# tudelft-iv/CCVPE

Measured on NVIDIA B200. Metric: VIGOR pairs/sec (CVM_VIGOR forward + pose decode, 320x640 panorama + 512x512 aerial), higher is better.
Workload: dtype bf16

## Files before the change

### ccvpe_b200/build.py

```python
from __future__ import annotations

import concurrent.futures
import os
import shutil
import subprocess
import sys

PKG_DIR = os.path.dirname(os.path.abspath(__file__))
CSRC = os.path.join(PKG_DIR, "csrc")
OBJ_DIR = os.path.join(PKG_DIR, "build")
INCLUDE = os.path.join(os.path.dirname(PKG_DIR), "include")
LIB_PATH = os.path.join(PKG_DIR, "libccvpe_b200.so")
SOURCES = ["runtime.cu", "descriptors.cu", "match.cu", "pointwise.cu", "igemm_simt.cu", "igemm_tcgen05.cu",
           "conv_ring_tcgen05.cu", "match_tcgen05.cu", "project_tcgen05.cu", "stem_tcgen05.cu", "encoder_ops.cu", "ingest.cu", "train_ops.cu", "wgrad_tcgen05.cu"]
NVCC_FLAGS = ["-gencode", "arch=compute_100a,code=sm_100a", "-lineinfo", "-O3", "-std=c++17", "-Xcompiler", "-fPIC"]


def _nvcc() -> str:
    for cand in (os.environ.get("NVCC"), shutil.which("nvcc"), "/usr/local/cuda/bin/nvcc"):
        if cand and os.path.exists(cand):
            return cand
    raise RuntimeError("nvcc not found; libccvpe_b200.so cannot be built")


def _headers():
    return [os.path.join(CSRC, f) for f in os.listdir(CSRC) if f.endswith((".cuh", ".h"))] + \
           [os.path.join(INCLUDE, "ccvpe_b200.h")]


def _sources():
    return [s for s in SOURCES if os.path.exists(os.path.join(CSRC, s))]


def stale() -> bool:
    if not os.path.exists(LIB_PATH):
        return True
    t = os.path.getmtime(LIB_PATH)
# ... 40 lines not shown
```

### ccvpe_b200/cabi.py

```python
from __future__ import annotations

import ctypes as C
import os
from typing import Optional, Sequence

import torch

from . import build as _build

F32, BF16 = 0, 1
ABI_VERSION = 3
SE_SUM_SCALE = 1048576.0
BACKEND_AUTO, BACKEND_SIMT, BACKEND_TCGEN05 = 0, 1, 2

EXPORTED_SYMBOLS = (
    "ccvpe_abi_version", "ccvpe_last_error", "ccvpe_launch_count", "ccvpe_reset_launch_count",
    "ccvpe_grd_descriptor", "ccvpe_grd_descriptors", "ccvpe_igemm", "ccvpe_igemm_plan", "ccvpe_match_scratch_elems", "ccvpe_match_plan", "ccvpe_match_level",
    "ccvpe_softmax_scratch_elems", "ccvpe_softmax_heatmap", "ccvpe_ori_normalize",
    "ccvpe_pose_scratch_bytes", "ccvpe_pose_decode", "ccvpe_bias_silu_nhwc", "ccvpe_dwconv_bias_silu_nhwc",
    "ccvpe_pointwise_silu_nhwc", "ccvpe_stem_conv_silu_nhwc", "ccvpe_se_gate_scale", "ccvpe_mbconv_project_nhwc",
    "ccvpe_wrap_columns_nhwc",
    "ccvpe_ingest_u8", "ccvpe_stem_conv_silu_u8_nhwc",
    "ccvpe_wgrad_workspace_elems", "ccvpe_wgrad", "ccvpe_wgrad_plan", "ccvpe_colsum_workspace_elems", "ccvpe_colsum",
    "ccvpe_relu_bwd", "ccvpe_scale_rows", "ccvpe_planar_to_cl", "ccvpe_cl_to_planar", "ccvpe_ori_normalize_bwd",
    "ccvpe_match_bwd_scratch_elems", "ccvpe_match_level_bwd", "ccvpe_loss_workspace_elems", "ccvpe_infonce_loss",
    "ccvpe_cross_entropy_loss", "ccvpe_orientation_loss", "ccvpe_grd_descriptors_bwd",
)


class CcvpeError(RuntimeError):
    pass


class IgemmDesc(C.Structure):
    _fields_ = [
        ("a0", C.c_void_p), ("a1", C.c_void_p),
        ("c0", C.c_int32), ("c1", C.c_int32), ("ld0", C.c_int32), ("ld1", C.c_int32),
        ("B", C.c_int32), ("Hin", C.c_int32), ("Win", C.c_int32), ("Hout", C.c_int32), ("Wout", C.c_int32),
        ("stride", C.c_int32), ("kh", C.c_int32), ("kw", C.c_int32), ("pad", C.c_int32),
        ("N", C.c_int32), ("dtype", C.c_int32),
        ("w_kn", C.c_void_p), ("w_nk", C.c_void_p),
        ("bias", C.c_void_p), ("row_scale", C.c_void_p), ("row_r1", C.c_void_p), ("r1_w", C.c_void_p),
        ("relu", C.c_int32), ("out_mode", C.c_int32), ("out_dtype", C.c_int32), ("ldo", C.c_int32),
        ("out", C.c_void_p),
# ... 75 lines not shown
    lib.ccvpe_bias_silu_nhwc.restype = C.c_int
    lib.ccvpe_bias_silu_nhwc.argtypes = [C.c_void_p, C.c_void_p, C.c_void_p, C.c_int64, C.c_int64, C.c_int64,
                                         C.c_int, C.c_int, C.c_int, C.c_int, C.c_void_p, C.c_void_p]
    lib.ccvpe_dwconv_bias_silu_nhwc.restype = C.c_int
    lib.ccvpe_dwconv_bias_silu_nhwc.argtypes = [C.c_void_p, C.c_int64, C.c_int64, C.c_int64, C.c_int, C.c_int,
                                                C.c_void_p, C.c_void_p, C.c_void_p, C.c_int, C.c_int, C.c_int, C.c_int,
                                                C.c_void_p, C.c_void_p]
    lib.ccvpe_pointwise_silu_nhwc.restype = C.c_int
    lib.ccvpe_pointwise_silu_nhwc.argtypes = [C.c_void_p, C.c_int, C.c_int, C.c_int, C.c_int, C.c_int, C.c_void_p,
                                              C.c_void_p, C.c_int, C.c_void_p, C.c_int, C.c_int, C.c_void_p]
    lib.ccvpe_stem_conv_silu_nhwc.restype = C.c_int
    lib.ccvpe_stem_conv_silu_nhwc.argtypes = [C.c_void_p, C.c_int, C.c_int, C.c_int, C.c_void_p, C.c_void_p, C.c_int,
                                              C.c_void_p, C.c_int, C.c_int, C.c_int, C.c_int, C.c_int, C.c_void_p]
    lib.ccvpe_stem_conv_silu_u8_nhwc.restype = C.c_int
    lib.ccvpe_stem_conv_silu_u8_nhwc.argtypes = [C.c_void_p, C.c_int, C.c_int, C.c_int, C.c_int, C.c_void_p,
                                                 C.POINTER(C.c_float), C.POINTER(C.c_float), C.c_void_p, C.c_void_p, C.c_int,
                                                 C.c_void_p, C.c_int, C.c_int, C.c_int, C.c_int, C.c_int, C.c_void_p]
    lib.ccvpe_se_gate_scale.restype = C.c_int
    lib.ccvpe_se_gate_scale.argtypes = [C.c_void_p, C.c_float] + [C.c_void_p] * 6 + [C.c_int] * 5 + [C.c_void_p] * 2
    lib.ccvpe_mbconv_project_nhwc.restype = C.c_int
    lib.ccvpe_mbconv_project_nhwc.argtypes = [C.c_void_p] * 6 + [C.c_int] * 4 + [C.c_void_p]
    lib.ccvpe_wrap_columns_nhwc.restype = C.c_int
    lib.ccvpe_wrap_columns_nhwc.argtypes = [C.c_void_p, C.c_int, C.c_int, C.c_int, C.c_int, C.c_int, C.c_int, C.c_void_p]
    lib.ccvpe_ingest_u8.restype = C.c_int
    lib.ccvpe_ingest_u8.argtypes = [C.c_void_p, C.c_int, C.c_int, C.c_int, C.c_int, C.c_int, C.c_void_p,
                                    C.POINTER(C.c_float), C.POINTER(C.c_float), C.c_void_p, C.c_void_p]
    lib.ccvpe_wgrad_workspace_elems.restype = C.c_int64
    lib.ccvpe_wgrad_workspace_elems.argtypes = [C.POINTER(WgradDesc)]
    lib.ccvpe_wgrad.restype = C.c_int
    lib.ccvpe_wgrad.argtypes = [C.POINTER(WgradDesc), C.c_void_p]
    lib.ccvpe_wgrad_plan.restype = C.c_int
    lib.ccvpe_wgrad_plan.argtypes = [C.POINTER(WgradDesc)]
    lib.ccvpe_colsum_workspace_elems.restype = C.c_int64
    lib.ccvpe_colsum_workspace_elems.argtypes = [C.c_int64, C.c_int, C.c_int]
    lib.ccvpe_colsum.restype = C.c_int
    lib.ccvpe_colsum.argtypes = [C.c_void_p, C.c_int, C.c_int, C.c_int, C.c_int, C.c_int, C.c_int, C.c_void_p, C.c_int,
                                 C.c_void_p, C.c_void_p, C.c_void_p]
    lib.ccvpe_relu_bwd.restype = C.c_int
    lib.ccvpe_relu_bwd.argtypes = [C.c_void_p, C.c_void_p, C.c_int, C.c_int64, C.c_void_p]
    lib.ccvpe_scale_rows.restype = C.c_int
    lib.ccvpe_scale_rows.argtypes = [C.c_void_p, C.c_int, C.c_void_p, C.c_void_p, C.c_int64, C.c_int, C.c_void_p]
    lib.ccvpe_planar_to_cl.restype = C.c_int
    lib.ccvpe_planar_to_cl.argtypes = [C.c_void_p, C.c_void_p, C.c_int, C.c_int, C.c_int, C.c_int64, C.c_int, C.c_void_p]
    lib.ccvpe_cl_to_planar.restype = C.c_int
    lib.ccvpe_cl_to_planar.argtypes = [C.c_void_p, C.c_int, C.c_void_p, C.c_int, C.c_int, C.c_int64, C.c_int, C.c_void_p]
    lib.ccvpe_ori_normalize_bwd.restype = C.c_int
# ... 202 lines not shown
                                       _ptr(chan_sum), _stream()), "ccvpe_bias_silu_nhwc")


def dwconv_bias_silu_nhwc(x_pad: torch.Tensor, w: torch.Tensor, bias: torch.Tensor, y: torch.Tensor, k: int, stride: int,
                          chan_sum: Optional[torch.Tensor] = None):
    _require_cuda(x_pad, w, bias, y, chan_sum)
    _check_se_sum(chan_sum)
    B, Hp, Wp, Cc = x_pad.shape
    if x_pad.stride(3) != 1 or not y.is_contiguous():
        raise CcvpeError("dwconv_bias_silu_nhwc: channels must be contiguous and y contiguous")
    _check(load().ccvpe_dwconv_bias_silu_nhwc(_ptr(x_pad), x_pad.stride(0), x_pad.stride(1), x_pad.stride(2), Hp, Wp,
                                              _ptr(w), _ptr(bias), _ptr(y), B, Cc, k, stride, _ptr(chan_sum), _stream()),
           "ccvpe_dwconv_bias_silu_nhwc")


def pad_k_blocks(w: torch.Tensor) -> torch.Tensor:
    N, K = w.shape
    kw = 16 if K <= 16 else (32 if K < 64 else 64)
    out = torch.zeros((N, -(-K // kw) * kw), dtype=torch.bfloat16, device=w.device)
    out[:, :K] = w
    return out.contiguous()


def pointwise_silu_nhwc(x: torch.Tensor, w_nk: torch.Tensor, bias: Optional[torch.Tensor], out: torch.Tensor,
                        pad_lo: int = 0, pad_hi: int = 0):
    _require_cuda(x, w_nk, bias, out)
    B, H, W, K = x.shape
    N = w_nk.shape[0]
    if not x.is_contiguous() or not out.is_contiguous() or x.dtype != torch.bfloat16 or out.dtype != torch.bfloat16:
        raise CcvpeError("pointwise_silu_nhwc: x and out must be contiguous bf16")
    if tuple(out.shape) != (B, H + pad_lo + pad_hi, W + pad_lo + pad_hi, N):
        raise CcvpeError(f"pointwise_silu_nhwc: out has shape {tuple(out.shape)}")
    if bias is not None and bias.dtype != torch.float32:
        raise CcvpeError("pointwise_silu_nhwc: bias must be fp32")
    _check(load().ccvpe_pointwise_silu_nhwc(_ptr(x), B, H, W, K, K, _ptr(w_nk), _ptr(bias), N, _ptr(out), pad_lo, pad_hi,
                                            _stream()), "ccvpe_pointwise_silu_nhwc")


def stem_conv_silu_nhwc(x: torch.Tensor, w: torch.Tensor, bias: torch.Tensor, out: torch.Tensor, in_pad_lo: int,
                        in_pad_hi: int, out_pad_lo: int, out_pad_hi: int, circular: bool):
    _require_cuda(x, w, bias, out)
    B, Cin, H, W = x.shape
    CO = w.shape[1]
    if Cin != 3 or x.dtype != torch.float32 or not x.is_contiguous() or w.dtype != torch.float32 or bias.dtype != torch.float32:
        raise CcvpeError("stem_conv_silu_nhwc: x must be contiguous fp32 [B,3,H,W], w / bias fp32")
    Ho, Wo = (H + in_pad_lo + in_pad_hi - 3) // 2 + 1, (W + in_pad_lo + in_pad_hi - 3) // 2 + 1
# ... 243 lines not shown
```

### ccvpe_b200/csrc/common.cuh

```cuda
#pragma once

#include <cuda_bf16.h>
#include <cuda_runtime.h>
#include <stdint.h>

#include <atomic>
#include <cstdarg>
#include <cstdio>

#include "../../include/ccvpe_b200.h"

namespace ccvpe {

char* last_error_buffer();
std::atomic<int64_t>& launch_counter();

inline int fail(int code, const char* fmt, ...) {
  va_list ap;
  va_start(ap, fmt);
  vsnprintf(last_error_buffer(), 512, fmt, ap);
  va_end(ap);
  return code;
}

// ... 67 lines not shown
  uint2 raw;
  raw.x = *reinterpret_cast<uint32_t*>(&lo);
  raw.y = *reinterpret_cast<uint32_t*>(&hi);
  *reinterpret_cast<uint2*>(p) = raw;
}

__device__ __forceinline__ uint64_t pack_f32x2(float lo, float hi) {
  uint64_t r;
  asm("mov.b64 %0, {%1, %2};" : "=l"(r) : "f"(lo), "f"(hi));
  return r;
}
__device__ __forceinline__ void unpack_f32x2(uint64_t v, float& lo, float& hi) {
  asm("mov.b64 {%0, %1}, %2;" : "=f"(lo), "=f"(hi) : "l"(v));
}
__device__ __forceinline__ uint64_t bf16x2_to_f32x2(uint32_t v) {
  return pack_f32x2(__uint_as_float(v << 16), __uint_as_float(v & 0xffff0000u));
}
__device__ __forceinline__ uint64_t ffma2(uint64_t a, uint64_t b, uint64_t c) {
  uint64_t d;
  asm("fma.rn.f32x2 %0, %1, %2, %3;" : "=l"(d) : "l"(a), "l"(b), "l"(c));
  return d;
}

__device__ __forceinline__ float warp_sum(float v) {
#pragma unroll
  for (int o = 16; o > 0; o >>= 1) v += __shfl_xor_sync(0xffffffffu, v, o);
  return v;
}
__device__ __forceinline__ float warp_max(float v) {
#pragma unroll
  for (int o = 16; o > 0; o >>= 1) v = fmaxf(v, __shfl_xor_sync(0xffffffffu, v, o));
  return v;
}

}
```

### ccvpe_b200/csrc/encoder_ops.cu

```cuda
#include <cstdlib>
#include <cstring>

#include "common.cuh"

namespace ccvpe {

constexpr float kSeFixedScale = 1048576.f;
__device__ __forceinline__ unsigned long long se_fixed(float v) {
  return (unsigned long long)__float2ll_rn(v * kSeFixedScale);
}

__global__ void __launch_bounds__(256)
bias_silu_nhwc_kernel(const __nv_bfloat16* __restrict__ x, const __nv_bfloat16* __restrict__ bias,
                      __nv_bfloat16* __restrict__ y, int64_t y_sb, int64_t y_sh, int64_t y_sw, int H, int W, int C,
                      int pix_per_block, long long* __restrict__ chan_sum) {
  extern __shared__ unsigned long long s_sum[];
  const int G = C >> 3;
  const int lanes = blockDim.x / G;
  const int cg = threadIdx.x % G, pl = threadIdx.x / G;
  const int b = blockIdx.y;
  const int HW = H * W;
  const int p_lo = blockIdx.x * pix_per_block;
  const int p_hi = min(HW, p_lo + pix_per_block);
  if (chan_sum) {
    for (int c = threadIdx.x; c < C; c += blockDim.x) s_sum[c] = 0ull;
    __syncthreads();
  }
  float bv[8] = {0.f, 0.f, 0.f, 0.f, 0.f, 0.f, 0.f, 0.f};
  if (bias && pl < lanes) {
    uint4 q = *reinterpret_cast<const uint4*>(bias + cg * 8);
    const __nv_bfloat162* h = reinterpret_cast<const __nv_bfloat162*>(&q);
#pragma unroll
    for (int j = 0; j < 4; ++j) {
// ... 804 lines not shown
```

### ccvpe_b200/fast_encoder.py

```python
from __future__ import annotations

from typing import Dict, List, Tuple

import torch
from torch.nn import functional as F

from . import cabi
from .efficientnet import EfficientNetB0, MBConv, SamePadConv2d


def _fold(conv: torch.nn.Conv2d, bn: torch.nn.BatchNorm2d) -> Tuple[torch.Tensor, torch.Tensor]:
    w = conv.weight.detach().float()
    scale = bn.weight.detach().float() / torch.sqrt(bn.running_var.detach().float() + bn.eps)
    bias = bn.bias.detach().float() - bn.running_mean.detach().float() * scale
    if conv.bias is not None:
        bias = bias + conv.bias.detach().float() * scale
    return w * scale.view(-1, 1, 1, 1), bias


class _Block:
    __slots__ = ("has_expand", "residual", "stride", "kernel", "pad_lo", "pad_hi", "w_exp", "b_exp", "w_exp_nk",
                 "b_exp_f32", "w_dw", "b_dw",
                 "w_red", "b_red", "w_se", "w_se_t", "b_se", "w_proj", "b_proj", "mid", "cout", "w_dw_taps")


class FastEncoder:
    def __init__(self, enc: EfficientNetB0, dtype: torch.dtype = torch.bfloat16):
        self.dtype = dtype
        self.circular = bool(enc._conv_stem._circular)
        dev = enc._conv_stem.weight.device
        cast = lambda t: t.to(device=dev, dtype=dtype).contiguous()
        w, b = _fold(enc._conv_stem, enc._bn0)
        self.stem_w = cast(w).contiguous(memory_format=torch.channels_last)
        self.stem_b = cast(b)
        self.stem_pad = (enc._conv_stem._pad_lo, enc._conv_stem._pad_hi)
        self.stem_w_taps = w.permute(1, 2, 3, 0).reshape(27, -1).to(device=dev, dtype=torch.float32).contiguous()
        self.stem_b_f32 = b.to(device=dev, dtype=torch.float32).contiguous()
        self.blocks: List[_Block] = []
        pending = None
        for blk in enc._blocks:
            assert isinstance(blk, MBConv)
            o = _Block()
            o.has_expand, o.residual = blk._has_expand, blk._residual
            dw: SamePadConv2d = blk._depthwise_conv
            o.stride, o.kernel = dw.stride[0], dw.kernel_size[0]
            o.pad_lo, o.pad_hi = dw._pad_lo, dw._pad_hi
            if o.has_expand:
                w, b = _fold(blk._expand_conv, blk._bn0)
                if pending is not None:
# ... 2 lines not shown
                o.w_exp_nk = cabi.pad_k_blocks(o.w_exp)
                o.b_exp_f32 = b.to(device=dev, dtype=torch.float32).contiguous()
            else:
                assert pending is None
                o.w_exp = o.b_exp = None
            w, b = _fold(dw, blk._bn1)
            o.w_dw, o.b_dw = cast(w).contiguous(memory_format=torch.channels_last), cast(b)
            o.mid = w.shape[0]
            o.w_dw_taps = cast(w.reshape(o.mid, -1).t())
            o.w_red, o.b_red = cast(blk._se_reduce.weight.detach().flatten(1)), cast(blk._se_reduce.bias.detach())
            o.w_se, o.b_se = cast(blk._se_expand.weight.detach().flatten(1)), cast(blk._se_expand.bias.detach())
            o.w_se_t = o.w_se.t().contiguous()
            w, b = _fold(blk._project_conv, blk._bn2)
            pending = b + (pending if (o.residual and pending is not None) else 0.0)
            o.w_proj, o.b_proj = cast(w.flatten(1)), cast(pending)
            o.cout = w.shape[0]
            self.blocks.append(o)
        w, b = _fold(enc._conv_head, enc._bn1)
        b = b + w.flatten(1) @ pending.to(w.device)
        self.head_w, self.head_b = cast(w.flatten(1)), cast(b)
        self.head_w_nk = cabi.pad_k_blocks(self.head_w)
        self.head_b_f32 = b.to(device=dev, dtype=torch.float32).contiguous()
        self._buffers: Dict[tuple, torch.Tensor] = {}
        self._mid_total = sum(o.mid for o in self.blocks)
        self.keep = set(range(len(self.blocks)))

    def _padded(self, B, C, H, W, lo, hi, tag) -> torch.Tensor:
        key = (tag, B, C, H, W, lo, hi)
        buf = self._buffers.get(key)
        if buf is None:
            buf = torch.zeros((B, H + lo + hi, W + lo + hi, C), dtype=self.dtype, device=self.stem_w.device)
            self._buffers[key] = buf
        return buf

    def _packed_bias(self, o, rep) -> torch.Tensor:
        key = ("bproj", id(o), rep)
        buf = self._buffers.get(key)
        if buf is None:
            buf = o.b_proj.repeat(rep).contiguous()
            self._buffers[key] = buf
        return buf

    def _wrap_columns(self, buf, H, W, lo, hi):
        if buf.is_cuda and buf.dtype == torch.bfloat16 and buf.is_contiguous():
            cabi.wrap_columns_nhwc(buf, H, W, lo, hi)
            return
        if lo:
            buf[:, lo:lo + H, :lo, :] = buf[:, lo:lo + H, W:W + lo, :]
        if hi:
            buf[:, lo:lo + H, lo + W:, :] = buf[:, lo:lo + H, lo:lo + hi, :]

    def _act(self, x_nhwc: torch.Tensor, bias, pad=None, want_sum: bool = False):
        B, H, W, C = x_nhwc.shape
        buf = None
        if pad is not None:
            lo, hi = pad
# ... 35 lines not shown
                cabi.stem_conv_silu_u8_nhwc(x.contiguous(), self.stem_w_taps, self.stem_b_f32, buf, lo, hi, o0.pad_lo,
                                            o0.pad_hi, self.circular)
            else:
                cabi.stem_conv_silu_nhwc(x.float().contiguous(), self.stem_w_taps, self.stem_b_f32, buf, lo, hi, o0.pad_lo,
                                         o0.pad_hi, self.circular)
            stem_padded = buf.permute(0, 3, 1, 2)
            pre = pre_bias = None
        else:
            if x.dtype == torch.uint8:
                raise cabi.CcvpeError("uint8 images are ingested by the CUDA bf16 encoder plan only (models.ingest otherwise)")
            x = x.to(dt).contiguous(memory_format=torch.channels_last)
            if self.circular:
                x = F.pad(F.pad(x, (lo, hi, 0, 0), mode="circular"), (0, 0, lo, hi))
            else:
                x = F.pad(x, (lo, hi, lo, hi))
            pre = F.conv2d(x, self.stem_w, None, stride=2).permute(0, 2, 3, 1)
            pre_bias = self.stem_b
        cur = None
        outs: List[torch.Tensor] = []
        sums_ws = torch.zeros(x.shape[0] * self._mid_total, dtype=torch.int64, device=x.device) if fused_dw else None
        sums_off = 0
        for o in self.blocks:
            dw_pad = (o.pad_lo, o.pad_hi) if (self.circular or o.stride == 2 or fused_dw) else None
            if stem_padded is not None:
                block_in = None
                mid_in_plain, mid_in_padded = None, stem_padded
                stem_padded = None
            elif pre is not None and not o.has_expand and not o.residual:
                plain, padded, _unused = self._act(pre, pre_bias, pad=dw_pad)
                block_in = None
                mid_in_plain, mid_in_padded = (plain if padded is None else None), padded
                pre = None
            else:
                if pre is not None:
                    cur = self._act(pre, pre_bias)[0]
                    pre = None
                block_in = cur
                B, H, W, Cin = cur.shape
                if o.has_expand and fused_dw:
                    buf = self._padded(B, o.mid, H, W, o.pad_lo, o.pad_hi, "dw")
                    cabi.pointwise_silu_nhwc(cur, o.w_exp_nk, o.b_exp_f32, buf, o.pad_lo, o.pad_hi)
                    if self.circular:
                        self._wrap_columns(buf, H, W, o.pad_lo, o.pad_hi)
                    mid_in_plain, mid_in_padded = None, buf.permute(0, 3, 1, 2)
                elif o.has_expand:
                    e = F.linear(cur.reshape(B * H * W, Cin), o.w_exp, o.b_exp).view(B, H, W, o.mid)
                    plain, padded, _unused = self._act(e, None, pad=dw_pad)
                    mid_in_plain, mid_in_padded = (plain if padded is None else None), padded
                else:
                    if dw_pad is not None:
                        buf = self._padded(B, o.mid, H, W, o.pad_lo, o.pad_hi, "dw")
                        buf[:, o.pad_lo:o.pad_lo + H, o.pad_lo:o.pad_lo + W, :] = cur
                        if self.circular:
                            self._wrap_columns(buf, H, W, o.pad_lo, o.pad_hi)
                        mid_in_plain, mid_in_padded = None, buf.permute(0, 3, 1, 2)
                    else:
                        mid_in_plain, mid_in_padded = cur, None
            if fused_dw:
                xp = mid_in_padded.permute(0, 2, 3, 1)
                Bp, Hp, Wp, _ = xp.shape
                Ho, Wo = (Hp - o.kernel) // o.stride + 1, (Wp - o.kernel) // o.stride + 1
                d = torch.empty((Bp, Ho, Wo, o.mid), dtype=dt, device=xp.device)
                sums = sums_ws[sums_off:sums_off + Bp * o.mid].view(Bp, o.mid)
                sums_off += Bp * o.mid
                cabi.dwconv_bias_silu_nhwc(xp, o.w_dw_taps, o.b_dw, d, o.kernel, o.stride, sums)
            else:
                if mid_in_padded is not None:
                    d = F.conv2d(mid_in_padded, o.w_dw, None, stride=o.stride, groups=o.mid)
                else:
                    d = F.conv2d(mid_in_plain.permute(0, 3, 1, 2), o.w_dw, None, stride=1, padding=o.pad_lo,
                                 groups=o.mid)
                d, _unused, sums = self._act(d.permute(0, 2, 3, 1), o.b_dw, want_sum=True)
            Bo, Ho, Wo, _ = d.shape
            if fused_dw:
                rep = 2 if (o.mid <= 32 and (Ho * Wo) % 2 == 0 and not o.residual) else 1
                wg = torch.empty((Bo, rep * o.cout, rep * o.mid), dtype=dt, device=d.device)
                gate_ws = torch.empty((Bo, o.mid), dtype=torch.float32, device=d.device)
                cabi.se_gate_scale(sums, 1.0 / float(Ho * Wo), o.w_red, o.b_red, o.w_se_t, o.b_se, o.w_proj, wg, gate_ws, rep)
            else:
                sq = (sums / float(Ho * Wo)).to(dt)
                g = torch.sigmoid(F.linear(F.silu(F.linear(sq, o.w_red, o.b_red)), o.w_se, o.b_se))
# ... 39 lines not shown
```

### include/ccvpe_b200.h

```cpp
#ifndef CCVPE_B200_H_
#define CCVPE_B200_H_

#include <stdint.h>

#ifdef __cplusplus
extern "C" {
#endif

#define CCVPE_ABI_VERSION 3

enum { CCVPE_F32 = 0, CCVPE_BF16 = 1 };

enum {
  CCVPE_OK = 0,
  CCVPE_ERR_BAD_ARGUMENT = -1,
  CCVPE_ERR_UNSUPPORTED = -2,
  CCVPE_ERR_CUDA = -3,
  CCVPE_ERR_NO_DEVICE = -4
};

enum {
  CCVPE_BACKEND_AUTO = 0,
  CCVPE_BACKEND_SIMT = 1,
  CCVPE_BACKEND_TCGEN05 = 2
// ... 61 lines not shown

int ccvpe_dwconv_bias_silu_nhwc(const void* x, int64_t x_sb, int64_t x_sh, int64_t x_sw, int Hp, int Wp,
                                const void* w, const void* bias, void* y, int B, int C, int K, int S,
                                int64_t* chan_sum, void* stream);

int ccvpe_stem_conv_silu_nhwc(const float* x, int B, int H, int W, const float* w, const float* bias, int CO,
                              void* out, int in_pad_lo, int in_pad_hi, int out_pad_lo, int out_pad_hi, int circular,
                              void* stream);

int ccvpe_stem_conv_silu_u8_nhwc(const uint8_t* x, int B, int H, int Wsrc, int crop_w, const int32_t* shift,
                                 const float* mean_host, const float* std_host, const float* w, const float* bias, int CO,
                                 void* out, int in_pad_lo, int in_pad_hi, int out_pad_lo, int out_pad_hi, int circular,
                                 void* stream);

int ccvpe_wrap_columns_nhwc(void* buf, int B, int H, int W, int C, int pad_lo, int pad_hi, void* stream);

int ccvpe_se_gate_scale(const int64_t* chan_sum, float inv_hw, const void* w_red, const void* b_red, const void* w_se,
                        const void* b_se, const void* w_proj, void* wg, int B, int mid, int R, int cout, int rep,
                        float* gate_ws, void* stream);

int ccvpe_pointwise_silu_nhwc(const void* x, int B, int H, int W, int K, int ldx, const void* w_nk, const float* bias,
                              int N, void* out, int pad_lo, int pad_hi, void* stream);

int ccvpe_mbconv_project_nhwc(const void* d, const void* wg, const void* residual, const void* bias, void* out,
                              void* out_biased, int B, int HW, int mid, int cout, void* stream);

int ccvpe_ingest_u8(const uint8_t* src, int nhwc, int B, int H, int W, int crop_w, const int32_t* shift,
                    const float* mean_host, const float* std_host, float* dst, void* stream);


typedef struct ccvpe_wgrad_desc {
  const void* a0; const void* a1;
  int32_t c0, c1, ld0, ld1;
  int32_t B, Hin, Win, Hout, Wout;
  int32_t stride, kh, kw, pad;
  const void* g; int32_t N, ldg;
  const float* g_row_scale;
  int32_t dtype;
  float* out;
  float* workspace; int64_t workspace_elems;
  int32_t backend;
} ccvpe_wgrad_desc;
int64_t ccvpe_wgrad_workspace_elems(const ccvpe_wgrad_desc* desc);
int ccvpe_wgrad(const ccvpe_wgrad_desc* desc, void* stream);
int ccvpe_wgrad_plan(const ccvpe_wgrad_desc* desc);

// ... 37 lines not shown
```

Baseline: 5958.

## Fuse MBConv expand 1x1 GEMM with depthwise conv in one tcgen05 kernel

Adds a persistent kernel that runs the 1x1 expansion GEMM on tcgen05 into TMEM, applies bias+SiLU, and writes rows into a shared-memory ring. Depthwise KxK conv, bias/SiLU and SE channel sums are then computed from that ring in the same kernel. This removes the round trip of the wide expanded activation through global memory and the separate launches for the early, narrow-input blocks. It costs heavy shared-memory use and redundant halo-row GEMM work between bands, and it applies only when Cin<=64 and mid is divisible by 48.

```diff
diff --git a/ccvpe_b200/build.py b/ccvpe_b200/build.py
--- a/ccvpe_b200/build.py
+++ b/ccvpe_b200/build.py
@@ -12,7 +12,7 @@
 INCLUDE = os.path.join(os.path.dirname(PKG_DIR), "include")
 LIB_PATH = os.path.join(PKG_DIR, "libccvpe_b200.so")
 SOURCES = ["runtime.cu", "descriptors.cu", "match.cu", "pointwise.cu", "igemm_simt.cu", "igemm_tcgen05.cu",
-           "conv_ring_tcgen05.cu", "match_tcgen05.cu", "project_tcgen05.cu", "stem_tcgen05.cu", "encoder_ops.cu", "ingest.cu", "train_ops.cu", "wgrad_tcgen05.cu"]
+           "conv_ring_tcgen05.cu", "match_tcgen05.cu", "project_tcgen05.cu", "stem_tcgen05.cu", "expand_dw_tcgen05.cu", "encoder_ops.cu", "ingest.cu", "train_ops.cu", "wgrad_tcgen05.cu"]
 NVCC_FLAGS = ["-gencode", "arch=compute_100a,code=sm_100a", "-lineinfo", "-O3", "-std=c++17", "-Xcompiler", "-fPIC"]
 
 
diff --git a/ccvpe_b200/cabi.py b/ccvpe_b200/cabi.py
--- a/ccvpe_b200/cabi.py
+++ b/ccvpe_b200/cabi.py
@@ -19,7 +19,7 @@
     "ccvpe_softmax_scratch_elems", "ccvpe_softmax_heatmap", "ccvpe_ori_normalize",
     "ccvpe_pose_scratch_bytes", "ccvpe_pose_decode", "ccvpe_bias_silu_nhwc", "ccvpe_dwconv_bias_silu_nhwc",
     "ccvpe_pointwise_silu_nhwc", "ccvpe_stem_conv_silu_nhwc", "ccvpe_se_gate_scale", "ccvpe_mbconv_project_nhwc",
-    "ccvpe_wrap_columns_nhwc",
+    "ccvpe_wrap_columns_nhwc", "ccvpe_mbconv_expand_dw_nhwc", "ccvpe_mbconv_expand_dw_supported",
     "ccvpe_ingest_u8", "ccvpe_stem_conv_silu_u8_nhwc",
     "ccvpe_wgrad_workspace_elems", "ccvpe_wgrad", "ccvpe_wgrad_plan", "ccvpe_colsum_workspace_elems", "ccvpe_colsum",
     "ccvpe_relu_bwd", "ccvpe_scale_rows", "ccvpe_planar_to_cl", "ccvpe_cl_to_planar", "ccvpe_ori_normalize_bwd",
@@ -141,6 +141,11 @@
     lib.ccvpe_mbconv_project_nhwc.argtypes = [C.c_void_p] * 6 + [C.c_int] * 4 + [C.c_void_p]
     lib.ccvpe_wrap_columns_nhwc.restype = C.c_int
     lib.ccvpe_wrap_columns_nhwc.argtypes = [C.c_void_p, C.c_int, C.c_int, C.c_int, C.c_int, C.c_int, C.c_int, C.c_void_p]
+    lib.ccvpe_mbconv_expand_dw_nhwc.restype = C.c_int
+    lib.ccvpe_mbconv_expand_dw_nhwc.argtypes = ([C.c_void_p] + [C.c_int] * 4 + [C.c_void_p, C.c_int, C.c_void_p, C.c_int]
+                                                + [C.c_void_p] * 2 + [C.c_int] * 5 + [C.c_void_p] * 3)
+    lib.ccvpe_mbconv_expand_dw_supported.restype = C.c_int
+    lib.ccvpe_mbconv_expand_dw_supported.argtypes = [C.c_int] * 11
     lib.ccvpe_ingest_u8.restype = C.c_int
     lib.ccvpe_ingest_u8.argtypes = [C.c_void_p, C.c_int, C.c_int, C.c_int, C.c_int, C.c_int, C.c_void_p,
                                     C.POINTER(C.c_float), C.POINTER(C.c_float), C.c_void_p, C.c_void_p]
@@ -389,6 +394,30 @@
     return out.contiguous()
 
 
+def mbconv_expand_dw_supported(B: int, H: int, W: int, cin: int, ldw: int, mid: int, k: int, stride: int, pad_lo: int,
+                               pad_hi: int, circular: bool) -> bool:
+    return bool(load().ccvpe_mbconv_expand_dw_supported(B, H, W, cin, ldw, mid, k, stride, pad_lo, pad_hi, int(circular)))
+
+
+def mbconv_expand_dw_nhwc(x: torch.Tensor, w_nk: torch.Tensor, b_e: torch.Tensor, w_dw: torch.Tensor, b_dw: torch.Tensor,
+                          y: torch.Tensor, k: int, stride: int, pad_lo: int, pad_hi: int, circular: bool,
+                          chan_sum: Optional[torch.Tensor] = None):
+    _require_cuda(x, w_nk, b_e, w_dw, b_dw, y, chan_sum)
+    _check_se_sum(chan_sum)
+    B, H, W, cin = x.shape
+    mid = w_nk.shape[0]
+    Ho, Wo = (H + pad_lo + pad_hi - k) // stride + 1, (W + pad_lo + pad_hi - k) // stride + 1
+    if any(t.dtype != torch.bfloat16 or not t.is_contiguous() for t in (x, w_nk, w_dw, b_dw, y)):
+        raise CcvpeError("mbconv_expand_dw_nhwc: x, w_nk, w_dw, b_dw and y must be contiguous bf16")
+    if b_e.dtype != torch.float32 or not b_e.is_contiguous():
+        raise CcvpeError("mbconv_expand_dw_nhwc: b_e must be contiguous fp32")
+    if tuple(y.shape) != (B, Ho, Wo, mid) or tuple(w_dw.shape) != (k * k, mid):
+        raise CcvpeError(f"mbconv_expand_dw_nhwc: y {tuple(y.shape)} / w_dw {tuple(w_dw.shape)} do not match")
+    _check(load().ccvpe_mbconv_expand_dw_nhwc(_ptr(x), B, H, W, cin, _ptr(w_nk), w_nk.shape[1], _ptr(b_e), mid, _ptr(w_dw),
+                                              _ptr(b_dw), k, stride, pad_lo, pad_hi, int(circular), _ptr(y),
+                                              _ptr(chan_sum), _stream()), "ccvpe_mbconv_expand_dw_nhwc")
+
+
 def pointwise_silu_nhwc(x: torch.Tensor, w_nk: torch.Tensor, bias: Optional[torch.Tensor], out: torch.Tensor,
                         pad_lo: int = 0, pad_hi: int = 0):
     _require_cuda(x, w_nk, bias, out)
diff --git a/ccvpe_b200/csrc/common.cuh b/ccvpe_b200/csrc/common.cuh
--- a/ccvpe_b200/csrc/common.cuh
+++ b/ccvpe_b200/csrc/common.cuh
@@ -113,6 +113,11 @@
   return d;
 }
 
+constexpr float kSeFixedScale = 1048576.f;
+__device__ __forceinline__ unsigned long long se_fixed(float v) {
+  return (unsigned long long)__float2ll_rn(v * kSeFixedScale);
+}
+
 __device__ __forceinline__ float warp_sum(float v) {
 #pragma unroll
   for (int o = 16; o > 0; o >>= 1) v += __shfl_xor_sync(0xffffffffu, v, o);
diff --git a/ccvpe_b200/csrc/encoder_ops.cu b/ccvpe_b200/csrc/encoder_ops.cu
--- a/ccvpe_b200/csrc/encoder_ops.cu
+++ b/ccvpe_b200/csrc/encoder_ops.cu
@@ -4,11 +4,6 @@
 #include "common.cuh"
 
 namespace ccvpe {
-
-constexpr float kSeFixedScale = 1048576.f;
-__device__ __forceinline__ unsigned long long se_fixed(float v) {
-  return (unsigned long long)__float2ll_rn(v * kSeFixedScale);
-}
 
 __global__ void __launch_bounds__(256)
 bias_silu_nhwc_kernel(const __nv_bfloat16* __restrict__ x, const __nv_bfloat16* __restrict__ bias,
diff --git a/ccvpe_b200/csrc/expand_dw_tcgen05.cu b/ccvpe_b200/csrc/expand_dw_tcgen05.cu
--- /dev/null
+++ b/ccvpe_b200/csrc/expand_dw_tcgen05.cu
@@ -0,0 +1,508 @@
+#include <array>
+#include <cstring>
+#include <map>
+#include <mutex>
+
+#include "tcgen05_common.cuh"
+
+namespace ccvpe {
+
+constexpr int XDW_THREADS = 256;
+constexpr int XDW_NC = 48;
+constexpr int XDW_PIX_BYTES = XDW_NC * 2;
+constexpr int XDW_CG = XDW_NC / 4;
+constexpr int XDW_LANES = XDW_THREADS / XDW_CG;
+constexpr int XDW_TW = 4;
+constexpr int XDW_A_SLICE = TC_BM * 32;
+constexpr int XDW_B_SLICE = XDW_NC * 32;
+constexpr int XDW_TMEM_COLS = 128;
+constexpr int XDW_SMEM_LIMIT = 226 * 1024;
+
+struct ExpandDwParams {
+  const __nv_bfloat16* x;
+  const __nv_bfloat16* w_nk;
+  const float* b_e;
+  const __nv_bfloat16* w_dw;
+  const __nv_bfloat16* b_dw;
+  __nv_bfloat16* y;
+  long long* chan_sum;
+  int B, H, W, Cin, ldw, mid, pad_lo, Wp, Ho, Wo;
+  int ksl, strips, nchunks, BH, nbands, DR, ring, total_items;
+  int na;
+  int off_b, off_wdw, off_bdw, off_be, off_part, off_ring;
+  int fills;
+};
+
+__device__ __forceinline__ void xdw_cp_async16(uint32_t dst, const void* src, uint32_t src_bytes) {
+  asm volatile("cp.async.cg.shared.global [%0], [%1], 16, %2;" ::"r"(dst), "l"(src), "r"(src_bytes) : "memory");
+}
+__device__ __forceinline__ void xdw_tmem_ld16(uint32_t taddr, uint32_t* r) {
+  asm volatile(
+      "tcgen05.ld.sync.aligned.32x32b.x16.b32 "
+      "{%0, %1, %2, %3, %4, %5, %6, %7, %8, %9, %10, %11, %12, %13, %14, %15}, [%16];"
+      : "=r"(r[0]), "=r"(r[1]), "=r"(r[2]), "=r"(r[3]), "=r"(r[4]), "=r"(r[5]), "=r"(r[6]), "=r"(r[7]), "=r"(r[8]),
+        "=r"(r[9]), "=r"(r[10]), "=r"(r[11]), "=r"(r[12]), "=r"(r[13]), "=r"(r[14]), "=r"(r[15])
+      : "r"(taddr)
+      : "memory");
+}
+__device__ __forceinline__ void xdw_tmem_ld8(uint32_t taddr, uint32_t* r) {
+  asm volatile("tcgen05.ld.sync.aligned.32x32b.x8.b32 {%0, %1, %2, %3, %4, %5, %6, %7}, [%8];"
+               : "=r"(r[0]), "=r"(r[1]), "=r"(r[2]), "=r"(r[3]), "=r"(r[4]), "=r"(r[5]), "=r"(r[6]), "=r"(r[7])
+               : "r"(taddr)
+               : "memory");
+}
+__device__ __forceinline__ uint2 xdw_lds64(uint32_t addr) {
+  uint2 v;
+  asm volatile("ld.shared.v2.u32 {%0, %1}, [%2];" : "=r"(v.x), "=r"(v.y) : "r"(addr));
+  return v;
+}
+
+template <int K, int S, bool CIRC>
+__global__ void __launch_bounds__(XDW_THREADS) expand_dw_kernel(const __grid_constant__ ExpandDwParams p) {
+  constexpr int IW = (XDW_TW - 1) * S + K;
+  extern __shared__ __align__(16) uint8_t smem_raw[];
+  __shared__ __align__(8) uint64_t bar[2];
+  __shared__ uint32_t tmem_slot;
+
+  const int tid = threadIdx.x, warp = tid >> 5, lane = tid & 31;
+  const uint32_t s_base = (smem_u32(smem_raw) + 1023u) & ~1023u;
+  uint8_t* smem = smem_raw + (s_base - smem_u32(smem_raw));
+  const uint32_t s_a = s_base, s_b = s_base + p.off_b, s_wdw = s_base + p.off_wdw, s_ring = s_base + p.off_ring;
+  const __nv_bfloat16* s_bdw = reinterpret_cast<const __nv_bfloat16*>(smem + p.off_bdw);
+  float* s_be = reinterpret_cast<float*>(smem + p.off_be);
+  float* s_part = reinterpret_cast<float*>(smem + p.off_part);
+  uint8_t* ring = smem + p.off_ring;
+  const int slot_bytes = p.Wp * XDW_PIX_BYTES;
+  const int a_stage = p.ksl * XDW_A_SLICE;
+
+  for (int i = tid; i < p.na * TC_BM * 2 * p.ksl; i += XDW_THREADS) {
+    const int c = i % (2 * p.ksl), q = i / (2 * p.ksl), row = q % TC_BM, st = q / TC_BM;
+    if (c * 8 >= p.Cin)
+      *reinterpret_cast<uint4*>(smem + st * a_stage + (c >> 1) * XDW_A_SLICE + row * 32 +
+                                (((c & 1) ^ ((row >> 2) & 1)) << 4)) = make_uint4(0u, 0u, 0u, 0u);
+  }
+  if (!CIRC) {
+    const int bw = p.Wp - p.W;
+    for (int i = tid; i < p.ring * bw * (XDW_PIX_BYTES / 16); i += XDW_THREADS) {
+      const int v = i % (XDW_PIX_BYTES / 16), q = i / (XDW_PIX_BYTES / 16), cb = q % bw, slot = q / bw;
+      const int col = cb < p.pad_lo ? cb : p.W + cb;
+      *reinterpret_cast<uint4*>(ring + slot * slot_bytes + col * XDW_PIX_BYTES + v * 16) = make_uint4(0u, 0u, 0u, 0u);
+    }
+  }
+  if (tid == 0) {
+    mbar_init(smem_u32(&bar[0]), 1);
+    mbar_init(smem_u32(&bar[1]), 1);
+    asm volatile("fence.mbarrier_init.release.cluster;" ::: "memory");
+  }
+  if (warp == 0) {
+    asm volatile("tcgen05.alloc.cta_group::1.sync.aligned.shared::cta.b32 [%0], %1;" ::"r"(smem_u32(&tmem_slot)),
+                 "r"(XDW_TMEM_COLS) : "memory");
+    asm volatile("tcgen05.relinquish_alloc_permit.cta_group::1.sync.aligned;" ::: "memory");
+  }
+  tc_fence_before();
+  __syncthreads();
+  tc_fence_after();
+  const uint32_t tmem_base = tmem_slot;
+
+  const uint32_t idesc = (1u << 4) | (1u << 7) | (1u << 10) | ((uint32_t)(XDW_NC >> 3) << 17) | ((uint32_t)(TC_BM >> 4) << 24);
+  const uint64_t dhi = make_smem_desc(0, 16) & 0xFFFFFFFF00000000ull;
+  auto desc = [&](uint32_t addr) -> uint64_t { return dhi | (((addr & 0x3FFFFu) >> 4) | (1u << 16)); };
+
+  const int cg = tid % XDW_CG, pl = tid / XDW_CG;
+  const int nstr = (p.Wo + XDW_TW - 1) / XDW_TW;
+  uint32_t g = 0;
+
+  for (int item = blockIdx.x; item < p.total_items; item += gridDim.x) {
+    const int chunk = item % p.nchunks;
+    const int band = (item / p.nchunks) % p.nbands;
+    const int b = item / (p.nchunks * p.nbands);
+    const int c0 = chunk * XDW_NC;
+    const int ho_lo = band * p.BH, ho_hi = min(p.Ho, ho_lo + p.BH);
+    const int rp_lo = ho_lo * S, rp_hi = (ho_hi - 1) * S + K;
+    const int h_lo = max(0, rp_lo - p.pad_lo), h_hi = min(p.H, rp_hi - p.pad_lo);
+    const int njobs = h_hi > h_lo ? (h_hi - h_lo) * p.strips : 0;
+    const __nv_bfloat16* xb = p.x + (int64_t)b * p.H * p.W * p.Cin;
+
+    for (int i = tid; i < XDW_NC * 2 * p.ksl; i += XDW_THREADS) {
+      const int n = i / (2 * p.ksl), c = i % (2 * p.ksl);
+      const uint4 v = __ldg(reinterpret_cast<const uint4*>(p.w_nk + (int64_t)(c0 + n) * p.ldw + c * 8));
+      *reinterpret_cast<uint4*>(smem + p.off_b + (c >> 1) * XDW_B_SLICE + n * 32 + (((c & 1) ^ ((n >> 2) & 1)) << 4)) = v;
+    }
+    for (int i = tid; i < K * K * (XDW_NC / 8); i += XDW_THREADS) {
+      const int tap = i / (XDW_NC / 8), v = i % (XDW_NC / 8);
+      *reinterpret_cast<uint4*>(smem + p.off_wdw + tap * XDW_PIX_BYTES + v * 16) =
+          __ldg(reinterpret_cast<const uint4*>(p.w_dw + (int64_t)tap * p.mid + c0) + v);
+    }
+    if (tid < XDW_NC / 8)
+      reinterpret_cast<uint4*>(smem + p.off_bdw)[tid] = __ldg(reinterpret_cast<const uint4*>(p.b_dw + c0) + tid);
+    if (tid < XDW_NC) s_be[tid] = 0.5f * __ldg(p.b_e + c0 + tid);
+
+    auto load_a = [&](int j) {
+      const int h = h_lo + j / p.strips, w0 = (j % p.strips) * TC_BM;
+      const int row = tid & (TC_BM - 1);
+      const int w = w0 + row;
+      const bool ok = w < p.W;
+      const __nv_bfloat16* src = xb + ((int64_t)h * p.W + (ok ? w : 0)) * p.Cin;
+      const uint32_t dst = s_a + (uint32_t)(((g + j) % p.na) * a_stage) + row * 32;
+      for (int c = tid >> 7; c * 8 < p.Cin; c += 2)
+        xdw_cp_async16(dst + (c >> 1) * XDW_A_SLICE + (((c & 1) ^ ((row >> 2) & 1)) << 4), src + c * 8, ok ? 16u : 0u);
+      asm volatile("cp.async.commit_group;" ::: "memory");
+    };
+    auto mma = [&](int j) {
+      const int pending = min(njobs - 1, j + p.na - 2) - j;
+      if (pending >= 2) asm volatile("cp.async.wait_group 2;" ::: "memory");
+      else if (pending == 1) asm volatile("cp.async.wait_group 1;" ::: "memory");
+      else asm volatile("cp.async.wait_group 0;" ::: "memory");
+      asm volatile("fence.proxy.async.shared::cta;" ::: "memory");
+      tc_fence_before();
+      __syncthreads();
+      tc_fence_after();
+      if (warp == 0) {
+        if (elect_one()) {
+          const uint32_t s = (g + j) & 1;
+          const uint32_t a = s_a + ((g + j) % p.na) * a_stage;
+          for (int k = 0; k < p.ksl; ++k)
+            umma_bf16(tmem_base + s * 64, desc(a + k * XDW_A_SLICE), desc(s_b + k * XDW_B_SLICE), idesc, k > 0 ? 1u : 0u);
+          umma_commit(smem_u32(&bar[s]));
+        }
+        __syncwarp();
+      }
+    };
+    auto epilogue = [&](int j, int slot) {
+      const uint32_t s = (g + j) & 1;
+      mbar_wait(smem_u32(&bar[s]), ((g + j) >> 1) & 1);
+      tc_fence_after();
+      const int half = warp >> 2;
+      const int ca = half * 16, cb = 32 + half * 8;
+      const uint32_t taddr = tmem_base + ((uint32_t)((warp & 3) * 32) << 16) + s * 64;
+      uint32_t v[24];
+      xdw_tmem_ld16(taddr + ca, v);
+      xdw_tmem_ld8(taddr + cb, v + 16);
+      tmem_ld_wait();
+      tc_fence_before();
+      if (j + p.na < njobs) load_a(j + p.na);
+      const int w = (j % p.strips) * TC_BM + (warp & 3) * 32 + lane;
+      if (w >= p.W) return;
+      uint4 o[3];
+      __nv_bfloat162* hv = reinterpret_cast<__nv_bfloat162*>(o);
+#pragma unroll
+      for (int c = 0; c < 24; c += 2) {
+        const int ch = c < 16 ? ca + c : cb + c - 16;
+        const float a0 = fmaf(__uint_as_float(v[c]), 0.5f, s_be[ch]);
+        const float a1 = fmaf(__uint_as_float(v[c + 1]), 0.5f, s_be[ch + 1]);
+        hv[c >> 1] = __floats2bfloat162_rn(fmaf(a0, tanh_approx(a0), a0), fmaf(a1, tanh_approx(a1), a1));
+      }
+      uint8_t* srow = ring + slot * slot_bytes;
+      auto put = [&](int col) {
+        uint8_t* px = srow + col * XDW_PIX_BYTES;
+        reinterpret_cast<uint4*>(px + ca * 2)[0] = o[0];
+        reinterpret_cast<uint4*>(px + ca * 2)[1] = o[1];
+        *reinterpret_cast<uint4*>(px + cb * 2) = o[2];
+      };
+      put(p.pad_lo + w);
+      if (CIRC) {
+        if (w >= p.W - p.pad_lo) put(w - (p.W - p.pad_lo));
+        if (w < p.Wp - p.pad_lo - p.W) put(p.pad_lo + p.W + w);
+      }
+    };
+
+    float csum[4] = {0.f, 0.f, 0.f, 0.f};
+    auto depthwise = [&](int o_lo, int o_hi) {
+      if (pl >= XDW_LANES) return;
+      uint64_t bv[2];
+      {
+        const uint2 bq = *reinterpret_cast<const uint2*>(s_bdw + cg * 4);
+        bv[0] = bf16x2_to_f32x2(bq.x);
+        bv[1] = bf16x2_to_f32x2(bq.y);
+      }
+      const int nq = (o_hi - o_lo) * nstr;
+      for (int q = pl; q < nq; q += XDW_LANES) {
+        const int ho = o_lo + q / nstr, wo0 = (q % nstr) * XDW_TW;
+        uint64_t acc[XDW_TW][2];
+#pragma unroll
+        for (int t = 0; t < XDW_TW; ++t) {
+          acc[t][0] = bv[0];
+          acc[t][1] = bv[1];
+        }
+#pragma unroll
+        for (int ky = 0; ky < K; ++ky) {
+          const int slot = (ho * S + ky - rp_lo) % p.ring;
+          const uint32_t srow = s_ring + (uint32_t)(slot * slot_bytes) + cg * 8;
+          uint2 xin[IW];
+#pragma unroll
+          for (int ix = 0; ix < IW; ++ix)
+            xin[ix] = xdw_lds64(srow + (uint32_t)(min(wo0 * S + ix, p.Wp - 1) * XDW_PIX_BYTES));
+          uint64_t xf[IW][2];
+#pragma unroll
+          for (int ix = 0; ix < IW; ++ix) {
+            xf[ix][0] = bf16x2_to_f32x2(xin[ix].x);
+            xf[ix][1] = bf16x2_to_f32x2(xin[ix].y);
+          }
+#pragma unroll
+          for (int kx = 0; kx < K; ++kx) {
+            const uint2 wq = xdw_lds64(s_wdw + (uint32_t)((ky * K + kx) * XDW_PIX_BYTES) + cg * 8);
+            const uint64_t w0 = bf16x2_to_f32x2(wq.x), w1 = bf16x2_to_f32x2(wq.y);
+#pragma unroll
+            for (int t = 0; t < XDW_TW; ++t) {
+              acc[t][0] = ffma2(xf[t * S + kx][0], w0, acc[t][0]);
+              acc[t][1] = ffma2(xf[t * S + kx][1], w1, acc[t][1]);
+            }
+          }
+        }
+        __nv_bfloat16* yrow = p.y + (((int64_t)b * p.Ho + ho) * p.Wo) * p.mid + c0 + cg * 4;
+#pragma unroll
+        for (int t = 0; t < XDW_TW; ++t) {
+          const int wo = wo0 + t;
+          if (wo < p.Wo) {
+            uint2 qv;
+            __nv_bfloat162* hq = reinterpret_cast<__nv_bfloat162*>(&qv);
+#pragma unroll
+            for (int jj = 0; jj < 2; ++jj) {
+              float a0, a1;
+              unpack_f32x2(acc[t][jj], a0, a1);
+              a0 *= 0.5f;
+              a1 *= 0.5f;
+              a0 = fmaf(a0, tanh_approx(a0), a0);
+              a1 = fmaf(a1, tanh_approx(a1), a1);
+              hq[jj] = __floats2bfloat162_rn(a0, a1);
+              const float2 r = __bfloat1622float2(hq[jj]);
+              csum[2 * jj] += r.x;
+              csum[2 * jj + 1] += r.y;
+            }
+            *reinterpret_cast<uint2*>(yrow + (int64_t)wo * p.mid) = qv;
+          }
+        }
+      }
+    };
+
+    for (int j = 0; j < p.na && j < njobs; ++j) load_a(j);
+    if (njobs > 0) mma(0);
+    int je = 0, o_next = ho_lo;
+    for (int rp = rp_lo; rp < rp_hi; ++rp) {
+      const int slot = (rp - rp_lo) % p.ring;
+      const int h = rp - p.pad_lo;
+      if (h >= 0 && h < p.H) {
+        for (int st = 0; st < p.strips; ++st, ++je) {
+          if (je + 1 < njobs) mma(je + 1);
+          epilogue(je, slot);
+        }
+      } else {
+        for (int i = tid; i < slot_bytes / 16; i += XDW_THREADS)
+          reinterpret_cast<uint4*>(ring + slot * slot_bytes)[i] = make_uint4(0u, 0u, 0u, 0u);
+      }
+      const int o_end = min(o_next + p.DR, ho_hi);
+      if (rp == (o_end - 1) * S + K - 1) {
+        __syncthreads();
+        depthwise(o_next, o_end);
+        __syncthreads();
+        o_next = o_end;
+      }
+    }
+    g += (uint32_t)njobs;
+
+    if (p.chan_sum) {
+      if (pl < XDW_LANES) {
+#pragma unroll
+        for (int jj = 0; jj < 4; ++jj) s_part[pl * XDW_NC + cg * 4 + jj] = csum[jj];
+      }
+      __syncthreads();
+      if (tid < XDW_NC) {
+        float tot = 0.f;
+        for (int l = 0; l < XDW_LANES; ++l) tot += s_part[l * XDW_NC + tid];
+        atomicAdd(reinterpret_cast<unsigned long long*>(p.chan_sum) + (int64_t)b * p.mid + c0 + tid, se_fixed(tot));
+      }
+      __syncthreads();
+    }
+  }
+
+  tc_fence_before();
+  __syncthreads();
+  if (warp == 0) {
+    tc_fence_after();
+    asm volatile("tcgen05.dealloc.cta_group::1.sync.aligned.b32 %0, %1;" ::"r"(tmem_base), "r"(XDW_TMEM_COLS) : "memory");
+  }
+}
+
+template <int K, int S, bool CIRC>
+static const void* xdw_fn() {
+  return reinterpret_cast<const void*>(&expand_dw_kernel<K, S, CIRC>);
+}
+static const void* xdw_select(int K, int S, bool circ) {
+  if (K == 3 && S == 1) return circ ? xdw_fn<3, 1, true>() : xdw_fn<3, 1, false>();
+  if (K == 3) return circ ? xdw_fn<3, 2, true>() : xdw_fn<3, 2, false>();
+  if (S == 1) return circ ? xdw_fn<5, 1, true>() : xdw_fn<5, 1, false>();
+  return circ ? xdw_fn<5, 2, true>() : xdw_fn<5, 2, false>();
+}
+
+static int xdw_smem_bytes(const ExpandDwParams& p) { return 1024 + p.off_ring + p.ring * p.Wp * XDW_PIX_BYTES; }
+
+static int xdw_plan_uncached(ExpandDwParams* p, int K, int S, bool circ, int* grid) {
+  const int sms = sm_count();
+  p->ksl = (p->Cin + 15) / 16;
+  p->strips = (p->W + TC_BM - 1) / TC_BM;
+  p->nchunks = p->mid / XDW_NC;
+  auto layout = [&](ExpandDwParams* q, int na) {
+    int off = na * q->ksl * XDW_A_SLICE;
+    q->na = na;
+    q->off_b = off;          off += q->ksl * XDW_B_SLICE;
+    q->off_wdw = off;        off += K * K * XDW_PIX_BYTES;
+    q->off_bdw = off;        off += XDW_PIX_BYTES;
+    q->off_be = off;         off += XDW_NC * 4;
+    q->off_part = off;       off += XDW_LANES * XDW_NC * 4;
+    q->off_ring = (off + 127) & ~127;
+  };
+  const int slot_bytes = p->Wp * XDW_PIX_BYTES;
+  const int nstr = (p->Wo + XDW_TW - 1) / XDW_TW;
+  const void* fn = xdw_select(K, S, circ);
+  static thread_local uint64_t attr_set = 0;
+  if (first_use_on_device(attr_set)) {
+    for (int k = 3; k <= 5; k += 2)
+      for (int s = 1; s <= 2; ++s)
+        for (int c = 0; c < 2; ++c)
+          if (cudaFuncSetAttribute(xdw_select(k, s, c != 0), cudaFuncAttributeMaxDynamicSharedMemorySize,
+                                   XDW_SMEM_LIMIT) != cudaSuccess)
+            return fail(CCVPE_ERR_CUDA, "expand_dw: cudaFuncSetAttribute failed");
+  }
+  double best = 1e300;
+  bool found = false;
+  for (int DR = 1; DR <= 8 && DR <= p->Ho; ++DR) {
+    const int ring = (DR - 1) * S + K;
+    int occ = 0, na = 0;
+    ExpandDwParams lay = *p;
+    for (int n = 2; n <= 4; ++n) {
+      ExpandDwParams q = *p;
+      layout(&q, n);
+      const int smem = 1024 + q.off_ring + ring * slot_bytes;
+      int o = 0;
+      if (smem > XDW_SMEM_LIMIT ||
+          cudaOccupancyMaxActiveBlocksPerMultiprocessor(&o, fn, XDW_THREADS, smem) != cudaSuccess || o < 1)
+        break;
+      if (o > 512 / XDW_TMEM_COLS) o = 512 / XDW_TMEM_COLS;
+      if (n > 2 && o < occ) break;
+      occ = o;
+      na = n;
+      lay = q;
+    }
+    if (na == 0) break;
+    const int slots = occ * sms;
+    const int units = DR * nstr;
+    const double util = (double)units / (double)(((units + XDW_LANES - 1) / XDW_LANES) * XDW_LANES);
+    for (int nb = 1; nb <= p->Ho; ++nb) {
+      int BH = (p->Ho + nb - 1) / nb;
+      BH = (BH + DR - 1) / DR * DR;
+      const int nbands = (p->Ho + BH - 1) / BH;
+      if (nbands != nb) continue;
+      const int64_t items = (int64_t)p->B * nbands * p->nchunks;
+      if (items >= (1LL << 30)) continue;
+      const double item_cost = ((BH - 1) * S + K) * (double)p->W + BH * (double)p->Wo * (1.0 + K * K / 8.0) / util;
+      const double waves = (double)((items + slots - 1) / slots);
+      const double cost = waves * item_cost * occ / (occ >= 2 ? 1.0 : 0.6);
+      const bool fills = items >= sms;
+      if ((fills && !p->fills) || (fills == (bool)p->fills && cost < best)) {
+        best = cost;
+        p->fills = fills ? 1 : 0;
+        found = true;
+        p->na = lay.na;
+        p->off_b = lay.off_b; p->off_wdw = lay.off_wdw; p->off_bdw = lay.off_bdw;
+        p->off_be = lay.off_be; p->off_part = lay.off_part; p->off_ring = lay.off_ring;
+        p->DR = DR;
+        p->ring = ring;
+        p->BH = BH;
+        p->nbands = nbands;
+        p->total_items = (int)items;
+        *grid = (int)(items < slots ? items : slots);
+      }
+    }
+  }
+  return found ? CCVPE_OK : fail(CCVPE_ERR_UNSUPPORTED, "expand_dw: no shared-memory plan for Wp=%d", p->Wp);
+}
+
+static int xdw_plan(ExpandDwParams* p, int K, int S, bool circ, int* grid) {
+  struct Plan {
+    int rc, grid;
+    ExpandDwParams p;
+  };
+  static std::mutex mu;
+  static std::map<std::array<int, 12>, Plan> cache;
+  int dev = 0;
+  cudaGetDevice(&dev);
+  const std::array<int, 12> key = {dev, p->B, p->H, p->W, p->Cin, p->ldw, p->mid, K, S, p->pad_lo, p->Wp, circ ? 1 : 0};
+  {
+    std::lock_guard<std::mutex> lk(mu);
+    auto it = cache.find(key);
+    if (it != cache.end()) {
+      *p = it->second.p;
+      *grid = it->second.grid;
+      return it->second.rc == CCVPE_OK ? CCVPE_OK : fail(it->second.rc, "expand_dw: no shared-memory plan for Wp=%d", p->Wp);
+    }
+  }
+  Plan pl;
+  pl.grid = 0;
+  pl.rc = xdw_plan_uncached(p, K, S, circ, &pl.grid);
+  if (pl.rc == CCVPE_ERR_CUDA) return pl.rc;
+  pl.p = *p;
+  *grid = pl.grid;
+  std::lock_guard<std::mutex> lk(mu);
+  cache[key] = pl;
+  return pl.rc;
+}
+
+static int xdw_fill(ExpandDwParams* p, int B, int H, int W, int Cin, int ldw, int mid, int K, int S, int pad_lo,
+                    int pad_hi, int circular) {
+  if (B <= 0 || H <= 0 || W <= 0 || Cin <= 0 || Cin > 64 || Cin % 8 != 0 || mid <= 0 || mid % XDW_NC != 0 ||
+      (K != 3 && K != 5) || (S != 1 && S != 2) || pad_lo < 0 || pad_hi < 0 || pad_lo >= K || pad_hi >= K ||
+      ldw < (Cin + 15) / 16 * 16 || ldw % 8 != 0 || (circular && (pad_lo > W || pad_hi > W)))
+    return fail(CCVPE_ERR_UNSUPPORTED,
+                "expand_dw: B=%d H=%d W=%d Cin=%d ldw=%d mid=%d K=%d S=%d pad=(%d,%d) unsupported (Cin <= 64, mid %% 48 == 0)",
+                B, H, W, Cin, ldw, mid, K, S, pad_lo, pad_hi);
+  memset(p, 0, sizeof(*p));
+  p->B = B; p->H = H; p->W = W; p->Cin = Cin; p->ldw = ldw; p->mid = mid; p->pad_lo = pad_lo;
+  p->Wp = W + pad_lo + pad_hi;
+  const int Hp = H + pad_lo + pad_hi;
+  if (Hp < K || p->Wp < K) return fail(CCVPE_ERR_UNSUPPORTED, "expand_dw: image smaller than the window");
+  p->Ho = (Hp - K) / S + 1;
+  p->Wo = (p->Wp - K) / S + 1;
+  if ((int64_t)B * H * W * Cin >= (1LL << 40)) return fail(CCVPE_ERR_UNSUPPORTED, "expand_dw: input too large");
+  return CCVPE_OK;
+}
+
+}
+
+extern "C" int ccvpe_mbconv_expand_dw_supported(int B, int H, int W, int Cin, int ldw, int mid, int K, int S, int pad_lo,
+                                                int pad_hi, int circular) {
+  using namespace ccvpe;
+  ExpandDwParams p;
+  int grid = 0;
+  if (xdw_fill(&p, B, H, W, Cin, ldw, mid, K, S, pad_lo, pad_hi, circular) != CCVPE_OK) return 0;
+  return xdw_plan(&p, K, S, circular != 0, &grid) == CCVPE_OK && p.fills ? 1 : 0;
+}
+
+extern "C" int ccvpe_mbconv_expand_dw_nhwc(const void* x, int B, int H, int W, int Cin, const void* w_nk, int ldw,
+                                           const float* b_e, int mid, const void* w_dw, const void* b_dw, int K, int S,
+                                           int pad_lo, int pad_hi, int circular, void* y, int64_t* chan_sum,
+                                           void* stream) {
+  using namespace ccvpe;
+  CCVPE_REQUIRE(x && w_nk && b_e && w_dw && b_dw && y, "ccvpe_mbconv_expand_dw_nhwc: null pointer");
+  CCVPE_REQUIRE(aligned16(x) && aligned16(w_nk) && aligned16(w_dw) && aligned16(b_dw) && aligned16(y),
+                "ccvpe_mbconv_expand_dw_nhwc: pointers must be 16-byte aligned");
+  ExpandDwParams p;
+  int rc = xdw_fill(&p, B, H, W, Cin, ldw, mid, K, S, pad_lo, pad_hi, circular);
+  if (rc != CCVPE_OK) return rc;
+  int grid = 0;
+  rc = xdw_plan(&p, K, S, circular != 0, &grid);
+  if (rc != CCVPE_OK) return rc;
+  p.x = (const __nv_bfloat16*)x; p.w_nk = (const __nv_bfloat16*)w_nk; p.b_e = b_e;
+  p.w_dw = (const __nv_bfloat16*)w_dw; p.b_dw = (const __nv_bfloat16*)b_dw; p.y = (__nv_bfloat16*)y;
+  p.chan_sum = reinterpret_cast<long long*>(chan_sum);
+  const int smem = xdw_smem_bytes(p);
+  cudaStream_t st = (cudaStream_t)stream;
+  const bool circ = circular != 0;
+#define CCVPE_XDW(KK, SS, CC) expand_dw_kernel<KK, SS, CC><<<grid, XDW_THREADS, smem, st>>>(p)
+  if (K == 3 && S == 1) { if (circ) { CCVPE_XDW(3, 1, true); } else { CCVPE_XDW(3, 1, false); } }
+  else if (K == 3) { if (circ) { CCVPE_XDW(3, 2, true); } else { CCVPE_XDW(3, 2, false); } }
+  else if (S == 1) { if (circ) { CCVPE_XDW(5, 1, true); } else { CCVPE_XDW(5, 1, false); } }
+  else { if (circ) { CCVPE_XDW(5, 2, true); } else { CCVPE_XDW(5, 2, false); } }
+#undef CCVPE_XDW
+  CCVPE_LAUNCH_CHECK("expand_dw_kernel");
+  return CCVPE_OK;
+}
diff --git a/ccvpe_b200/fast_encoder.py b/ccvpe_b200/fast_encoder.py
--- a/ccvpe_b200/fast_encoder.py
+++ b/ccvpe_b200/fast_encoder.py
@@ -25,6 +25,8 @@
 
 
 class FastEncoder:
+    fuse_expand_dw = True
+
     def __init__(self, enc: EfficientNetB0, dtype: torch.dtype = torch.bfloat16):
         self.dtype = dtype
         self.circular = bool(enc._conv_stem._circular)
@@ -73,6 +75,7 @@
         self.head_w_nk = cabi.pad_k_blocks(self.head_w)
         self.head_b_f32 = b.to(device=dev, dtype=torch.float32).contiguous()
         self._buffers: Dict[tuple, torch.Tensor] = {}
+        self._fused_ok: Dict[tuple, bool] = {}
         self._mid_total = sum(o.mid for o in self.blocks)
         self.keep = set(range(len(self.blocks)))
 
@@ -83,6 +86,17 @@
             buf = torch.zeros((B, H + lo + hi, W + lo + hi, C), dtype=self.dtype, device=self.stem_w.device)
             self._buffers[key] = buf
         return buf
+
+    def _fuse(self, o, B, H, W, Cin) -> bool:
+        if not self.fuse_expand_dw or Cin > 64:
+            return False
+        key = (id(o), B, H, W, torch.cuda.current_device())
+        ok = self._fused_ok.get(key)
+        if ok is None:
+            ok = cabi.mbconv_expand_dw_supported(B, H, W, Cin, o.w_exp_nk.shape[1], o.mid, o.kernel, o.stride, o.pad_lo,
+                                                 o.pad_hi, self.circular)
+            self._fused_ok[key] = ok
+        return ok
 
     def _packed_bias(self, o, rep) -> torch.Tensor:
         key = ("bproj", id(o), rep)
@@ -164,6 +178,7 @@
         sums_off = 0
         for o in self.blocks:
             dw_pad = (o.pad_lo, o.pad_hi) if (self.circular or o.stride == 2 or fused_dw) else None
+            d = None
             if stem_padded is not None:
                 block_in = None
                 mid_in_plain, mid_in_padded = None, stem_padded
@@ -179,7 +194,14 @@
                     pre = None
                 block_in = cur
                 B, H, W, Cin = cur.shape
-                if o.has_expand and fused_dw:
+                if o.has_expand and fused_dw and self._fuse(o, B, H, W, Cin):
+                    Ho, Wo = (H + o.pad_lo + o.pad_hi - o.kernel) // o.stride + 1, (W + o.pad_lo + o.pad_hi - o.kernel) // o.stride + 1
+                    d = torch.empty((B, Ho, Wo, o.mid), dtype=dt, device=cur.device)
+                    sums = sums_ws[sums_off:sums_off + B * o.mid].view(B, o.mid)
+                    sums_off += B * o.mid
+                    cabi.mbconv_expand_dw_nhwc(cur, o.w_exp_nk, o.b_exp_f32, o.w_dw_taps, o.b_dw, d, o.kernel, o.stride,
+                                               o.pad_lo, o.pad_hi, self.circular, sums)
+                elif o.has_expand and fused_dw:
                     buf = self._padded(B, o.mid, H, W, o.pad_lo, o.pad_hi, "dw")
                     cabi.pointwise_silu_nhwc(cur, o.w_exp_nk, o.b_exp_f32, buf, o.pad_lo, o.pad_hi)
                     if self.circular:
@@ -198,7 +220,9 @@
                         mid_in_plain, mid_in_padded = None, buf.permute(0, 3, 1, 2)
                     else:
                         mid_in_plain, mid_in_padded = cur, None
-            if fused_dw:
+            if d is not None:
+                pass
+            elif fused_dw:
                 xp = mid_in_padded.permute(0, 2, 3, 1)
                 Bp, Hp, Wp, _ = xp.shape
                 Ho, Wo = (Hp - o.kernel) // o.stride + 1, (Wp - o.kernel) // o.stride + 1
diff --git a/include/ccvpe_b200.h b/include/ccvpe_b200.h
--- a/include/ccvpe_b200.h
+++ b/include/ccvpe_b200.h
@@ -107,6 +107,12 @@
 int ccvpe_pointwise_silu_nhwc(const void* x, int B, int H, int W, int K, int ldx, const void* w_nk, const float* bias,
                               int N, void* out, int pad_lo, int pad_hi, void* stream);
 
+int ccvpe_mbconv_expand_dw_nhwc(const void* x, int B, int H, int W, int Cin, const void* w_nk, int ldw, const float* b_e,
+                                int mid, const void* w_dw, const void* b_dw, int K, int S, int pad_lo, int pad_hi,
+                                int circular, void* y, int64_t* chan_sum, void* stream);
+int ccvpe_mbconv_expand_dw_supported(int B, int H, int W, int Cin, int ldw, int mid, int K, int S, int pad_lo, int pad_hi,
+                                     int circular);
+
 int ccvpe_mbconv_project_nhwc(const void* d, const void* wg, const void* residual, const void* bias, void* out,
                               void* out_biased, int B, int HW, int mid, int cout, void* stream);
 
```

Measured after the change: 5186, median of 6. -12.9%, worse.
